# BurnhamG/PyTorch-ScalableFHVAE

Measured on AMD Instinct MI355X. Metric: segments/sec + ELBO (nats/frame), (B,20,80) fbank, higher is better.
Workload: dtype bf16; 1 GPU; c3: fhvae.FHVAE 2x256 LSTM enc/dec, z1=z2=32, 28k-seq mu2 table, batch 2048; per-GPU batch 2048, T=20, F=80, full train step (fwd+loss+bwd+Adam), intended objective, mu_idx uniform; global_batch=2048, parallelism=single

## Files before the change

### include/fhvae_hip.h

```cpp
#ifndef FHVAE_HIP_H
#define FHVAE_HIP_H

#include <stdint.h>

#ifdef __cplusplus
extern "C" {
#endif

#define FHVAE_ABI_VERSION 11

enum { FHVAE_F32 = 0, FHVAE_BF16 = 1 };

enum {
  FHVAE_OK = 0,
  FHVAE_ERR_NULL = -1,
  FHVAE_ERR_SHAPE = -2,
  FHVAE_ERR_DTYPE = -3,
  FHVAE_ERR_ALIGN = -4,
  FHVAE_ERR_LIMIT = -5
};

#define FHVAE_MAX_LAYERS 4
#define FHVAE_LSTM_SYNC_BYTES 16384

// ... 68 lines not shown
int64_t fhvae_lstm_ws_below_elems(const fhvae_lstm_desc* d);
int fhvae_lstm_form(const fhvae_lstm_desc* d);
int fhvae_lstm_seq_fwd(const fhvae_lstm_desc* d, void* stream);
int64_t fhvae_lstm_infer_cs_elems(const fhvae_lstm_desc* d);
int fhvae_lstm_seq_infer(const fhvae_lstm_desc* d, void* stream);

typedef struct fhvae_lstm_bwd_desc {
  fhvae_lstm_desc f;
  const float* d_hs_top;
  const float* d_hn;
  void* dgates;
  float* dgsum;
  float* dc;
  float* dw_ih[FHVAE_MAX_LAYERS];
  float* dw_hh[FHVAE_MAX_LAYERS];
  float* db_ih[FHVAE_MAX_LAYERS];
  float* db_hh[FHVAE_MAX_LAYERS];
  float* d_xc;
  int32_t phase;
  float* ws_below;
} fhvae_lstm_bwd_desc;

int fhvae_lstm_seq_bwd(const fhvae_lstm_bwd_desc* d, void* stream);
typedef struct fhvae_wgrad_desc {
  const void* a; int64_t lda;
  int64_t a_col0;
  const void* b; int64_t ldb;
  float* c; int64_t ldc;
  int64_t M, N, K;
} fhvae_wgrad_desc;
int fhvae_wgrad_desc_ok(const fhvae_wgrad_desc* p);
int fhvae_lstm_param_grads_multi(const fhvae_lstm_bwd_desc* const* descs, int n, const fhvae_wgrad_desc* extra, int n_extra,
                                 void* stream);
int fhvae_wgrad_bf16(const void* a, int64_t lda, const void* b, int64_t ldb, float* c, int64_t ldc, int64_t M,
                     int64_t N, int64_t K, void* stream);
int fhvae_wgrad_f32(const float* a, int64_t lda, const float* b, int64_t ldb, float* c, int64_t ldc, int64_t M, int64_t N,
                    int64_t K, void* stream);

int fhvae_proj_bf16(const void* a, int64_t lda, const void* b, int64_t ldb, const float* bias, float* c, int64_t ldc,
                    int64_t M, int64_t N, int64_t K, void* stream);

int fhvae_mu2_gather_fwd(const float* table, const int64_t* idx, int64_t idx_offset, float* mu2,
                         int64_t B, int64_t S, int64_t D, int32_t* oob_flag, void* stream);
int fhvae_mu2_gather_bwd(const float* dmu2, const int64_t* idx, int64_t idx_offset, float* dtable,
                         int64_t B, int64_t S, int64_t D, float scale, void* stream);

typedef struct fhvae_elbo_desc {
  int64_t B, T, F, D1, D2;
  const float* x;    int64_t x_sb, x_st;
  const float* x_mu; const float* x_lv; int64_t xo_sb, xo_st;
  const float* z1_mu; const float* z1_lv;
  const float* z2_mu; const float* z2_lv;
  const float* mu2;
  const int64_t* num_segs; double nsegs_scalar;
  float* lower_bound; float* log_px_z; float* neg_kld_z1; float* neg_kld_z2; float* log_pmu2;
} fhvae_elbo_desc;

int fhvae_elbo_fwd(const fhvae_elbo_desc* d, void* stream);

typedef struct fhvae_elbo_bwd_desc {
  fhvae_elbo_desc f;
  const float* g_lower_bound; const float* g_log_px_z; const float* g_neg_kld_z1;
  const float* g_neg_kld_z2; const float* g_log_pmu2;
  int32_t reference_detach;
  float* d_x_mu; float* d_x_lv;
  float* d_z1_mu; float* d_z1_lv; float* d_z2_mu; float* d_z2_lv; float* d_mu2;
// ... 85 lines not shown
```

### pytorch-scalablefhvae_amd/csrc/lstm.hip

```cpp
#include "gemm_launch.h"
#include "lstm_cell.h"
#include "lstm_cluster.h"
#include "wgrad.h"
#include "wgrad_f32.h"
#include <algorithm>
#include <vector>
#include "trace.h"
#include <cstdlib>

namespace fh {

constexpr int kCH = 32;

struct GateRowMap {
  int H;
  __device__ __forceinline__ int64_t operator()(int n) const {
    int unit = (n >> 6) * 16 + (n & 15);
    int gate = (n & 63) >> 4;
    return unit < H ? (int64_t)gate * H + unit : -1;
  }
  __device__ __forceinline__ bool all_valid(int n0, int n) const { return ((n0 + n) >> 6) * 16 <= H; }
};

template <typename T>
// ... 683 lines not shown
    return FHVAE_OK;
  }
  for (int64_t w = 0; w < T_ + L - 1; ++w) {
    int nj = 0;
    const BwdJobs<T> jobs = bwd_jobs<T>(bd, op, w, nj);
    double fl = 0;
    for (int j = 0; j < nj; ++j) fl += 2.0 * B * H * (jobs.job[j].seg[0].K + jobs.job[j].seg[1].K);
    const int ts = trace_begin(st, kTraceBwdCell, fl);
    const int bt = B >= 16384 ? 128 : 32;
    if (bt == 128) {
      dim3 grid((unsigned)fh_cdiv(B, 128), (unsigned)fh_cdiv(H, 64), (unsigned)nj);
      hipLaunchKernelGGL((lstm_bwd_step_kernel<T, 128, 64, 4, 1, 16>), grid, dim3(kThreads), 0, st, jobs);
    } else if (bt == 64) {
      dim3 grid((unsigned)fh_cdiv(B, 64), (unsigned)fh_cdiv(H, 64), (unsigned)nj);
      hipLaunchKernelGGL((lstm_bwd_step_kernel<T, 64, 64, 2, 2, 16>), grid, dim3(kThreads), 0, st, jobs);
    } else if (B >= 1024) {
      dim3 grid((unsigned)fh_cdiv(B, 32), (unsigned)fh_cdiv(H, 32), (unsigned)nj);
      hipLaunchKernelGGL((lstm_bwd_step_kernel<T, 32, 32, 2, 2, 16>), grid, dim3(kThreads), 0, st, jobs);
    } else {
      dim3 grid((unsigned)fh_cdiv(B, 32), (unsigned)fh_cdiv(H, 32), (unsigned)nj);
      hipLaunchKernelGGL((lstm_bwd_step_kernel<T, 32, 32, 2, 2, kCH>), grid, dim3(kThreads), 0, st, jobs);
    }
    trace_end(st, ts);
    int e = fh_launch_status();
    if (e) return e;
  }
  return FHVAE_OK;
}

constexpr int64_t kWgradMinK = 1024;

template <typename T>
static int lstm_param_grads(const fhvae_lstm_bwd_desc* bd, const Ops<T>& op, hipStream_t st, std::vector<WgProblem>* wq = nullptr,
                            std::vector<GemmParams>* fq = nullptr, std::vector<WgProblem32>* wq32 = nullptr) {
  const fhvae_lstm_desc* d = &bd->f;
  const int64_t B = d->B, T_ = d->T, I = d->I, Ic = d->Ic, H = d->H;
  const int L = d->L;
  const int64_t K0 = I + Ic, G = 4 * H;
  const T* dg = (const T*)bd->dgates;
  const T* hs = (const T*)d->hs;
  GemmParams grp[2 * FHVAE_MAX_LAYERS];
  int ng = 0;
  auto wgrad_long = [&](const void* a, int64_t lda, const void* b, int64_t ldb, int64_t Kc, float* c, int64_t ldc, int64_t Ncols) {
    if (sizeof(T) == 4) {
      if (!wq32 || Kc < kWgradMinK) return false;
      WgProblem32 w = {};
      w.A = (const float*)a, w.B = (const float*)b, w.C = c;
      w.lda = lda, w.ldb = ldb, w.ldc = ldc;
      w.M = (int)G, w.N = (int)Ncols, w.K = (int)Kc;
      if (!wgrad32_eligible(w)) return false;
      wq32->push_back(w);
      return true;
    }
    if (!wq || sizeof(T) != 2 || Kc < kWgradMinK) return false;
    WgProblem w = {};
    w.A = (const u16*)a, w.B = (const u16*)b, w.C = c;
    w.lda = lda, w.ldb = ldb, w.ldc = ldc;
    w.M = (int)G, w.N = (int)Ncols, w.K = (int)Kc;
    if (!wgrad_eligible(w)) return false;
    wq->push_back(w);
    return true;
  };
  auto wgrad = [&](const void* a, int64_t lda, const void* b, int64_t ldb, int64_t Kc, float* c, int64_t ldc, int64_t Ncols) {
    GemmParams p = {};
    p.seg[0] = Seg{a, lda, 0, b, ldb, 0, (int)Kc, 0};
    p.M = (int)G;
    p.N = (int)Ncols;
    p.C = c;
    p.ldc = ldc;
    p.splitk = 0;
    p.mode = 1;
    return p;
  };
  auto flush = [&]() -> int {
    int e = FHVAE_OK;
    for (int i = 0; i < ng && !e; i += kMaxGroup) e = launch_gemm_group(grp + i, ng - i < kMaxGroup ? ng - i : kMaxGroup, d->dtype, st);
    ng = 0;
    return e;
  };
  for (int l = 0; l < L; ++l) {
    const T* dgl = dg + (int64_t)l * T_ * B * G;
    const T* hl = hs + (int64_t)l * T_ * B * H;
    int e;
    if (bd->dw_hh[l] && T_ > 1 && !wgrad_long(dgl + B * G, G, hl, H, (T_ - 1) * B, bd->dw_hh[l], H, H))
      grp[ng++] = wgrad(dgl + B * G, G, hl, H, (T_ - 1) * B, bd->dw_hh[l], H, H);
    if (bd->dw_ih[l]) {
      if (l > 0) {
        if (!wgrad_long(dgl, G, hs + (int64_t)(l - 1) * T_ * B * H, H, T_ * B, bd->dw_ih[l], H, H))
          grp[ng++] = wgrad(dgl, G, hs + (int64_t)(l - 1) * T_ * B * H, H, T_ * B, bd->dw_ih[l], H, H);
      } else {
        if (I > 0 && !wgrad_long(dgl, G, op.x, I, T_ * B, bd->dw_ih[0], K0, I))
          grp[ng++] = wgrad(dgl, G, op.x, I, T_ * B, bd->dw_ih[0], K0, I);
        if (Ic > 0) {
          GemmParams p = wgrad(bd->dgsum, G, d->xc, Ic, B, bd->dw_ih[0] + I, K0, Ic);
          if (fq) {
            fq->push_back(p);
          } else {
            e = launch_gemm(p, FHVAE_F32, st);
            if (e) return e;
          }
        }
      }
    }
    if (!(sizeof(T) == 2 && cluster_eligible(d))) {
      if (l == 0 && Ic > 0 && bd->dgsum)
        e = launch_colsum(bd->dgsum, FHVAE_F32, G, bd->db_ih[l], bd->db_hh[l], B, G, st);
      else
        e = launch_colsum(dgl, d->dtype, G, bd->db_ih[l], bd->db_hh[l], T_ * B, G, st);
      if (e) return e;
    }
  }
  return flush();
}

static int lstm_dxc(const fhvae_lstm_bwd_desc* bd, hipStream_t st, bool zeroed = false) {
  const fhvae_lstm_desc* d = &bd->f;
  if (!bd->d_xc || d->Ic <= 0) return FHVAE_OK;
  const int64_t G = 4 * d->H, K0 = d->I + d->Ic;
  GemmParams p = {};
  p.seg[0] = Seg{bd->dgsum, G, 1, d->w_ih[0] + d->I, K0, 0, (int)G, 0};
  p.M = (int)d->B;
  p.N = (int)d->Ic;
  p.C = bd->d_xc;
  p.ldc = d->Ic;
  const int64_t tiles = fh_cdiv(d->B, 64) * fh_cdiv(d->Ic, 64);
  if (tiles <= 64 && G >= 512) {
    const int64_t n = d->B * d->Ic;
    if (!zeroed) hipLaunchKernelGGL(zero_f32_kernel, dim3((unsigned)fh_cdiv(n, 1024)), dim3(256), 0, st, bd->d_xc, n);
    p.mode = 2;
    int64_t sk = 256 / tiles;
    while (sk > 1 && G / sk < 128) sk >>= 1;
    p.splitk = (int)(sk < 4 ? 4 : sk > 16 ? 16 : sk);
  } else {
    p.splitk = 1;
  }
  return launch_gemm(p, FHVAE_F32, st);
}
// ... 25 lines not shown
    return launch_wgrad32(wq32.data(), (int)wq32.size(), st);
  }
  Ops<u16> op = ops_bf16(d);
  if (rec) {
    e = lstm_bwd_impl<u16>(bd, op, st);
    if (e) return e;
    e = lstm_dxc(bd, st, cluster_eligible(d) && cluster_bwd_zeroes_dxc(d));
    if (e) return e;
  }
  if (!par) return FHVAE_OK;
  std::vector<WgProblem> wq;
  e = lstm_param_grads<u16>(bd, op, st, getenv("FHVAE_NO_WGRAD") ? nullptr : &wq);
  if (e) return e;
  return launch_wgrad(wq.data(), (int)wq.size(), st);
}

static bool wg_from_desc(const fhvae_wgrad_desc* x, WgProblem& p) {
  if (!x || x->M <= 0 || x->N <= 0 || x->K <= 0 || x->M > INT32_MAX || x->N > INT32_MAX || x->K > INT32_MAX || x->a_col0 < 0 ||
      x->a_col0 > INT32_MAX)
    return false;
  p = WgProblem{};
  p.A = (const u16*)x->a, p.B = (const u16*)x->b, p.C = x->c;
  p.lda = x->lda, p.ldb = x->ldb, p.ldc = x->ldc;
  p.M = (int)x->M, p.N = (int)x->N, p.K = (int)x->K;
  p.a_col0 = (int)x->a_col0;
  return wgrad_eligible(p) && x->ldc >= x->N;
}

extern "C" int fhvae_wgrad_desc_ok(const fhvae_wgrad_desc* x) {
  WgProblem p;
  return wg_from_desc(x, p) ? 1 : 0;
}

extern "C" int fhvae_lstm_param_grads_multi(const fhvae_lstm_bwd_desc* const* bds, int n, const fhvae_wgrad_desc* extra, int n_extra,
                                            void* stream) {
  if (n < 0 || n_extra < 0) return FHVAE_ERR_SHAPE;
  if (n > 0) FH_CHECK_PTR(bds);
  if (n_extra > 0) FH_CHECK_PTR(extra);
  hipStream_t st = (hipStream_t)stream;
  std::vector<WgProblem> wq;
  for (int i = 0; i < n_extra; ++i) {
    WgProblem p;
    if (!wg_from_desc(extra + i, p)) return FHVAE_ERR_ALIGN;
    wq.push_back(p);
  }
  std::vector<GemmParams> fq;
  std::vector<WgProblem32> wq32;
  const bool use_wq = !getenv("FHVAE_NO_WGRAD");
  for (int i = 0; i < n; ++i) {
    const fhvae_lstm_bwd_desc* bd = bds[i];
    FH_CHECK_PTR(bd);
    const fhvae_lstm_desc* d = &bd->f;
    int e = check_desc(d);
    if (e) return e;
    FH_CHECK_PTR(bd->dgates);
    if (d->Ic > 0) FH_CHECK_PTR(bd->dgsum);
    if (d->dtype == FHVAE_F32) {
      e = lstm_param_grads<float>(bd, ops_f32(d), st, nullptr, nullptr, use_wq ? &wq32 : nullptr);
    } else {
      e = lstm_param_grads<u16>(bd, ops_bf16(d), st, use_wq ? &wq : nullptr, &fq);
    }
    if (e) return e;
  }
  for (size_t i = 0; i < fq.size();) {
    size_t j = i;
    while (j < fq.size() && j - i < (size_t)kMaxGroup) {
      bool dup = false;
      for (size_t k = i; k < j; ++k) dup = dup || fq[k].C == fq[j].C;
      if (dup) break;
      ++j;
    }
    const int e = launch_gemm_group(fq.data() + i, (int)(j - i), FHVAE_F32, st);
    if (e) return e;
    i = j;
  }
  {
    const int e = launch_wgrad32(wq32.data(), (int)wq32.size(), st);
    if (e) return e;
  }
  return launch_wgrad(wq.data(), (int)wq.size(), st);
}
```

### pytorch-scalablefhvae_amd/csrc/wgrad.h

```cpp
#pragma once
#include "common.h"

namespace fh {

struct WgProblem {
  const u16* A;
  const u16* B;
  float* C;
  int64_t lda, ldb, ldc;
  int M, N, K;
  int m_tiles, n_tiles, splitk, ksteps_per;
  int shared_c;
  int a_col0;
};

constexpr int kMaxWgProblems = 16;
struct WgGroup {
  int n;
  int base[kMaxWgProblems + 1];
  WgProblem p[kMaxWgProblems];
};

bool wgrad_eligible(const WgProblem& p);
int launch_wgrad(const WgProblem* ps, int n, hipStream_t st);

}
```

### pytorch-scalablefhvae_amd/csrc/wgrad.hip

```cpp
#include "wgrad.h"

#include <algorithm>
#include <cstdlib>

#include "gemm_core.h"

namespace fh {

constexpr int kWgThreads = 512;
constexpr int kWgBM = 256, kWgBK = 64;

template <int W>
struct WgImg {
  static constexpr int RB = W * 2;
  static constexpr int BYTES = kWgBK * RB;
  static constexpr int CPR = RB / 16;
  static constexpr int RPI = 1024 / RB;
  static constexpr int NI = BYTES / 1024 / 8;
};

typedef void __attribute__((address_space(3))) * lds_void_p;

template <int W>
__device__ __forceinline__ void wg_dma_offsets(unsigned (&voff)[WgImg<W>::NI], unsigned ld_bytes, int wave, int lane) {
  using I = WgImg<W>;
#pragma unroll
  for (int q = 0; q < I::NI; ++q) {
    const int row = (wave * I::NI + q) * I::RPI + lane / I::CPR;
    const int pc = lane % I::CPR;
    const int c = ((((pc >> 1) ^ (row & 7)) << 1) | (pc & 1));
    voff[q] = (unsigned)row * ld_bytes + (unsigned)c * 16u;
  }
}

template <int W>
__device__ __forceinline__ void wg_issue(char* stage, __amdgpu_buffer_rsrc_t rs, const unsigned (&voff)[WgImg<W>::NI], unsigned kbase,
                                         int wave) {
  using I = WgImg<W>;
#pragma unroll
  for (int q = 0; q < I::NI; ++q)
    __builtin_amdgcn_raw_ptr_buffer_load_lds(rs, (lds_void_p)(stage + (wave * I::NI + q) * 1024), 16, voff[q] + kbase, 0, 0, 0);
}

template <int RB>
__device__ __forceinline__ bf16x8 wg_frag(const char* img, int off, int j) {
  typedef s16x4 __attribute__((address_space(3))) * lds_p;
  const char* a0 = img + off + j * 32 * RB;
  union {
    struct {
      s16x4 lo, hi;
    } s;
    bf16x8 v;
  } u;
  u.s.lo = __builtin_amdgcn_ds_read_tr16_b64_v4i16((lds_p)(a0));
  u.s.hi = __builtin_amdgcn_ds_read_tr16_b64_v4i16((lds_p)(a0 + 16 * RB));
  return u.v;
}

template <int BN>
__global__ __launch_bounds__(kWgThreads) void wgrad_kernel(WgGroup g) {
  using IA = WgImg<kWgBM>;
  using IB = WgImg<BN>;
  constexpr int STAGE = IA::BYTES + IB::BYTES;
  constexpr int TM = 8, TN = BN / 64;
  constexpr int NLOAD = IA::NI + IB::NI;
  __shared__ __attribute__((aligned(1024))) char stage0[STAGE];
  __shared__ __attribute__((aligned(1024))) char stage1[STAGE];

  int wg = blockIdx.x;
  {
    const int nb = gridDim.x;
    if (nb >= 16) {
      const int q = nb >> 3, r = nb & 7, xcd = wg & 7;
      wg = (xcd < r ? xcd * (q + 1) : r * (q + 1) + (xcd - r) * q) + (wg >> 3);
    }
  }
  int pi = 0;
  while (pi + 1 < g.n && wg >= g.base[pi + 1]) ++pi;
  const WgProblem& p = g.p[pi];
  const int local = wg - g.base[pi];
  const int mt = local % p.m_tiles, nt = (local / p.m_tiles) % p.n_tiles, sp = local / (p.m_tiles * p.n_tiles);
  const int ks_total = (p.K + kWgBK - 1) / kWgBK;
  const int ks0 = sp * p.ksteps_per, ks1 = min(ks_total, ks0 + p.ksteps_per);
  if (ks0 >= ks1) return;
  const int m0 = mt * kWgBM, n0 = nt * BN;

  const int tid = threadIdx.x, lane = tid & 63, wave = tid >> 6;
  const int wm = wave >> 2, wn = wave & 3;
  const int gq = lane >> 4, i = lane & 15;

  const unsigned lda_b = (unsigned)p.lda * 2u, ldb_b = (unsigned)p.ldb * 2u;
  const __amdgpu_buffer_rsrc_t rsa =
      __builtin_amdgcn_make_buffer_rsrc(const_cast<u16*>(p.A + m0), 0, (int)(((int64_t)p.K * p.lda - p.a_col0 - m0) * 2), 0x00020000);
  const __amdgpu_buffer_rsrc_t rsb =
      __builtin_amdgcn_make_buffer_rsrc(const_cast<u16*>(p.B + n0), 0, (int)(((int64_t)p.K * p.ldb - n0) * 2), 0x00020000);
  unsigned va[IA::NI], vb[IB::NI];
  wg_dma_offsets<kWgBM>(va, lda_b, wave, lane);
  wg_dma_offsets<BN>(vb, ldb_b, wave, lane);
  auto a_step = [&](int ks) -> unsigned { return (unsigned)(ks * kWgBK) * lda_b; };

  const int kr = 4 * gq + (i >> 2), x = kr & 7;
  int offa[TM], offb[TN];
#pragma unroll
  for (int tm = 0; tm < TM; ++tm) offa[tm] = kr * IA::RB + ((((wm * 8 + tm)) ^ x) << 5) + 8 * (i & 3);
#pragma unroll
  for (int tn = 0; tn < TN; ++tn) offb[tn] = kr * IB::RB + ((((wn * TN + tn)) ^ x) << 5) + 8 * (i & 3);

  f32x4 acc[TM][TN];
#pragma unroll
  for (int tm = 0; tm < TM; ++tm)
#pragma unroll
    for (int tn = 0; tn < TN; ++tn) acc[tm][tn] = f32x4{0.f, 0.f, 0.f, 0.f};

  constexpr unsigned kOob = 0x40000000u;
  auto issue = [&](char* st, int ks) {
    const bool in = ks < ks1;
    wg_issue<kWgBM>(st, rsa, va, in ? a_step(ks) : kOob, wave);
// ... 6 lines not shown
      bf16x8 a[TM], b[TN];
#pragma unroll
      for (int tn = 0; tn < TN; ++tn) b[tn] = wg_frag<IB::RB>(Bs, offb[tn], j);
#pragma unroll
      for (int tm = 0; tm < TM; ++tm) a[tm] = wg_frag<IA::RB>(As, offa[tm], j);
      {
        const bool in = ks_next < ks1;
        if (j == 0)
          wg_issue<kWgBM>(nxt, rsa, va, in ? a_step(ks_next) : kOob, wave);
        else
          wg_issue<BN>(nxt + IA::BYTES, rsb, vb, in ? (unsigned)(ks_next * kWgBK) * ldb_b : kOob, wave);
      }
      __builtin_amdgcn_s_setprio(1);
#pragma unroll
      for (int tm = 0; tm < TM; ++tm)
#pragma unroll
        for (int tn = 0; tn < TN; ++tn) acc[tm][tn] = __builtin_amdgcn_mfma_f32_16x16x32_bf16(a[tm], b[tn], acc[tm][tn], 0, 0, 0);
      __builtin_amdgcn_s_setprio(0);
    }
  };
  auto step = [&](const char* cur, char* nxt, int ks_next) {
    asm volatile("s_waitcnt vmcnt(0)" ::: "memory");
    __builtin_amdgcn_s_barrier();
    compute(cur, nxt, ks_next);
    __builtin_amdgcn_s_barrier();
  };
  issue(stage0, ks0);
  for (int ks = ks0; ks < ks1; ks += 2) {
    step(stage0, stage1, ks + 1);
    step(stage1, stage0, ks + 2);
  }
  asm volatile("s_waitcnt vmcnt(0)" ::: "memory");

#pragma unroll
  for (int tm = 0; tm < TM; ++tm)
#pragma unroll
    for (int tn = 0; tn < TN; ++tn) {
      const int n = n0 + wn * (BN / 4) + tn * 16 + i;
#pragma unroll
      for (int r = 0; r < 4; ++r) {
        const int m = m0 + wm * 128 + tm * 16 + 4 * gq + r;
        if (m < p.M && n < p.N) {
          float* c = p.C + (int64_t)m * p.ldc + n;
          if (p.splitk == 1 && !p.shared_c)
            *c += acc[tm][tn][r];
          else
            atomicAdd(c, acc[tm][tn][r]);
        }
      }
    }
}

template __global__ void wgrad_kernel<256>(WgGroup);
template __global__ void wgrad_kernel<128>(WgGroup);

bool wgrad_eligible(const WgProblem& p) {
  if (p.M <= 0 || p.N <= 0 || p.K <= 0 || !p.A || !p.B || !p.C) return false;
  if ((((uintptr_t)p.A) | ((uintptr_t)p.B)) & 15) return false;
  if ((p.lda % 8) || (p.ldb % 8) || p.lda < p.a_col0 + p.M || p.ldb < p.N || p.a_col0 < 0) return false;
  if ((int64_t)p.K * p.lda * 2 >= (1LL << 30) || (int64_t)p.K * p.ldb * 2 >= (1LL << 30)) return false;
  return true;
}

template <int BN>
static int launch_class(const WgProblem* ps, const int* which, int n, hipStream_t st) {
  for (int at = 0; at < n; at += kMaxWgProblems) {
    const int cnt = n - at < kMaxWgProblems ? n - at : kMaxWgProblems;
    int64_t tiles = 0;
    for (int k = 0; k < cnt; ++k) {
      const WgProblem& p = ps[which[at + k]];
      tiles += fh_cdiv(p.M, kWgBM) * fh_cdiv(p.N, BN);
    }
    int64_t ks_max = 1;
    for (int k = 0; k < cnt; ++k) ks_max = std::max<int64_t>(ks_max, fh_cdiv(ps[which[at + k]].K, kWgBK));
    const double t_step = 2.0 * kWgBM * BN * kWgBK / (1.0e15 / 256), tile_bytes = 4.0 * kWgBM * BN;
    int64_t sk = 1;
    double best = 1e30;
    for (int64_t c = 1; c <= 64 && c * 2 <= ks_max; ++c) {
      const double waves = (double)fh_cdiv(tiles * c, 256), steps = (double)fh_cdiv(ks_max, c) + 2.0;
      const double t = waves * steps * t_step + (c > 1 ? tiles * c * tile_bytes / 1.3e12 : 0.0);
      if (t < best) best = t, sk = c;
    }
    WgGroup g = {};
    g.n = cnt;
    for (int k = 0; k < cnt; ++k) {
      WgProblem p = ps[which[at + k]];
      p.m_tiles = (int)fh_cdiv(p.M, kWgBM);
      p.n_tiles = (int)fh_cdiv(p.N, BN);
      const int64_t ks_total = fh_cdiv(p.K, kWgBK);
      int64_t s = sk;
      if (s > ks_total / 2) s = ks_total / 2;
      if (s < 1) s = 1;
      p.ksteps_per = (int)fh_cdiv(ks_total, s);
      p.splitk = (int)fh_cdiv(ks_total, p.ksteps_per);
      g.p[k] = p;
      g.base[k + 1] = g.base[k] + p.m_tiles * p.n_tiles * p.splitk;
    }
    for (int a = 0; a < cnt; ++a)
      for (int b = 0; b < cnt; ++b)
        if (a != b && g.p[a].C == g.p[b].C) g.p[a].shared_c = 1;
    const dim3 grid((unsigned)g.base[cnt]), block(kWgThreads);
    hipLaunchKernelGGL((wgrad_kernel<BN>), grid, block, 0, st, g);
    const int e = fh_launch_status();
    if (e) return e;
  }
  return FHVAE_OK;
}

int launch_wgrad(const WgProblem* ps, int n, hipStream_t st) {
  if (n <= 0) return FHVAE_OK;
  int wide[256], narrow[256], nw = 0, nn = 0;
  if (n > 256) return FHVAE_ERR_LIMIT;
  for (int k = 0; k < n; ++k) {
    if (!wgrad_eligible(ps[k])) return FHVAE_ERR_ALIGN;
    if (ps[k].N > 128)
      wide[nw++] = k;
    else
      narrow[nn++] = k;
  }
  int e = launch_class<256>(ps, wide, nw, st);
  if (e) return e;
  return launch_class<128>(ps, narrow, nn, st);
}

}

using namespace fh;

extern "C" int fhvae_wgrad_bf16(const void* a, int64_t lda, const void* b, int64_t ldb, float* c, int64_t ldc, int64_t M, int64_t N,
                                int64_t K, void* stream) {
  FH_CHECK_PTR(a);
  FH_CHECK_PTR(b);
  FH_CHECK_PTR(c);
  FH_CHECK_POS(M);
  FH_CHECK_POS(N);
  FH_CHECK_POS(K);
  FH_CHECK_I32(M);
  FH_CHECK_I32(N);
  FH_CHECK_I32(K);
  WgProblem p = {};
  p.A = (const u16*)a, p.B = (const u16*)b, p.C = c;
  p.lda = lda, p.ldb = ldb, p.ldc = ldc;
  p.M = (int)M, p.N = (int)N, p.K = (int)K;
  if (!wgrad_eligible(p)) return FHVAE_ERR_ALIGN;
  return launch_wgrad(&p, 1, (hipStream_t)stream);
}
```

### pytorch-scalablefhvae_amd/hip_binding.py

```python
from __future__ import annotations

import ctypes as C
import os
from typing import List, Optional, Sequence

import numpy as np
import torch

_HERE = os.path.dirname(os.path.abspath(__file__))
LIB_PATH = os.path.join(_HERE, "libfhvae_hip.so")

F32, BF16 = 0, 1
MAX_LAYERS = 4
ABI_VERSION = 11
PZ2_LOGVAR = np.log(0.5 ** 2).astype(np.float32)
INV_TWO_VAR = float(np.float32(1.0) / (np.float32(2.0) * np.exp(PZ2_LOGVAR)))

_vp, _i64, _i32, _f32, _f64 = C.c_void_p, C.c_int64, C.c_int32, C.c_float, C.c_double


class LstmDesc(C.Structure):
    _fields_ = [
        ("dtype", _i32), ("L", _i32),
        ("B", _i64), ("T", _i64), ("I", _i64), ("Ic", _i64), ("H", _i64),
# ... 43 lines not shown
class WgradDesc(C.Structure):
    _fields_ = [("a", _vp), ("lda", _i64), ("a_col0", _i64), ("b", _vp), ("ldb", _i64), ("c", _vp), ("ldc", _i64),
                ("M", _i64), ("N", _i64), ("K", _i64)]


SIGNATURES = {
    "fhvae_abi_version": (C.c_int, []),
    "fhvae_strerror": (C.c_char_p, [C.c_int]),
    "fhvae_linear_fwd": (C.c_int, [_vp, _i64, _vp, _i64, _vp, _vp, _i64, _vp, _i64, _i64, _i64, C.c_int, C.c_int, _vp]),
    "fhvae_linear_bwd": (C.c_int, [_vp, _i64, _vp, _i64, _vp, _i64, _vp, _i64, _vp, _vp, _i64, _vp, _i64, _vp, _i64, _i64,
                                   _i64, C.c_int, C.c_int, _vp]),
    "fhvae_gauss_head_reparam_fwd": (C.c_int, [_vp, _i64, _vp, _vp, _vp, _vp, _vp, _vp, _vp, _vp, _i64, _i64, _i64, C.c_int,
                                               _vp]),
    "fhvae_gauss_head_pair_fwd": (C.c_int, [_vp, _i64, _vp, _vp, _vp, _vp, _i64, _i64, _i64, _i64, _vp]),
    "fhvae_gauss_reparam_bwd": (C.c_int, [_vp, _vp, _vp, _vp, _vp, _vp, _vp, _i64, _vp]),
    "fhvae_gauss_head_bwd": (C.c_int, [_vp, _i64, _vp, _vp, _vp, _vp, _vp, _vp, _vp, _vp, _vp, _i64, _vp, _vp, _vp, _vp, _i64, _i64, _i64, _vp]),
    "fhvae_head_pair_weights": (C.c_int, [_vp, _vp, _vp, _vp, _i64, _i64, _i64, _vp]),
    "fhvae_gauss_reparam_pair_fwd": (C.c_int, [_vp, _i64, _vp, _vp, _vp, _vp, _i64, _i64, _vp]),
    "fhvae_gauss_reparam_bwd_pair": (C.c_int, [_vp, _vp, _vp, _i64, _vp, _vp, _i64, _vp, _i64, _vp, _vp, _i64, _i64, _vp]),
    "fhvae_elbo_colsum_rows": (_i64, [_i64]),
    "fhvae_gauss_head_bwd_pair": (C.c_int, [_vp, _i64, _vp, _i64, _vp, _i64, _vp, _i64, _vp, _i64, _vp, _vp, _vp, _vp, _i64, _i64, _i64, _vp]),
    "fhvae_loss_fwd": (C.c_int, [_vp, _vp, _f32, _vp, _i64, _vp, _vp]),
    "fhvae_loss_bwd": (C.c_int, [_vp, _f32, _vp, _vp, _i64, _vp]),
    "fhvae_lstm_lp_bytes": (_i64, [C.POINTER(LstmDesc)]),
    "fhvae_lstm_form": (C.c_int, [C.POINTER(LstmDesc)]),
    "fhvae_lstm_layout_id": (C.c_int, [C.POINTER(LstmDesc)]),
    "fhvae_lstm_pre_elems": (_i64, [C.POINTER(LstmDesc)]),
    "fhvae_lstm_ws_below_elems": (_i64, [C.POINTER(LstmDesc)]),
    "fhvae_lstm_seq_fwd": (C.c_int, [C.POINTER(LstmDesc), _vp]),
    "fhvae_lstm_infer_cs_elems": (_i64, [C.POINTER(LstmDesc)]),
    "fhvae_lstm_seq_infer": (C.c_int, [C.POINTER(LstmDesc), _vp]),
    "fhvae_lstm_seq_bwd": (C.c_int, [C.POINTER(LstmBwdDesc), _vp]),
    "fhvae_lstm_param_grads_multi": (C.c_int, [_vp, C.c_int, _vp, C.c_int, _vp]),
    "fhvae_wgrad_desc_ok": (C.c_int, [_vp]),
    "fhvae_wgrad_bf16": (C.c_int, [_vp, _i64, _vp, _i64, _vp, _i64, _i64, _i64, _i64, _vp]),
    "fhvae_wgrad_f32": (C.c_int, [_vp, _i64, _vp, _i64, _vp, _i64, _i64, _i64, _i64, _vp]),
    "fhvae_proj_bf16": (C.c_int, [_vp, _i64, _vp, _i64, _vp, _vp, _i64, _i64, _i64, _i64, _vp]),
    "fhvae_mu2_gather_fwd": (C.c_int, [_vp, _vp, _i64, _vp, _i64, _i64, _i64, _vp, _vp]),
    "fhvae_mu2_gather_bwd": (C.c_int, [_vp, _vp, _i64, _vp, _i64, _i64, _i64, _f32, _vp]),
    "fhvae_shard_pack": (C.c_int, [_vp, _vp, _vp, _i64, _i64, _vp]),
    "fhvae_shard_unpack": (C.c_int, [_vp, _vp, _vp, _i64, _i64, _vp]),
    "fhvae_disc_merge_partials": (C.c_int, [_vp, _vp, _vp, _vp, _i64, _i64, _vp]),
    "fhvae_shard_bwd_pack": (C.c_int, [_vp, _f32, _vp, _i64, _i64, _vp, _i64, _i64, _vp]),
    "fhvae_shard_bwd_unpack": (C.c_int, [_vp, _i64, _i64, _vp, _vp, _i64, _i64, _vp]),
    "fhvae_disc_ce_mean": (C.c_int, [_vp, _vp, _vp, _vp, _f32, _i64, _vp]),
    "fhvae_elbo_fwd": (C.c_int, [C.POINTER(ElboDesc), _vp]),
    "fhvae_elbo_bwd": (C.c_int, [C.POINTER(ElboBwdDesc), _vp]),
    "fhvae_disc_lse_ws_bytes": (_i64, [_i64, _i64]),
    "fhvae_disc_lse_bwd_ws_bytes": (_i64, [_i64, _i64, _i64]),
    "fhvae_disc_lse_fwd": (C.c_int, [_vp, _vp, _vp, _i64, _f32, _vp, _vp, _vp, _vp, _f32, _vp, _i64, _i64, _i64, C.c_int, _vp]),
    "fhvae_disc_lse_bwd": (C.c_int, [_vp, _vp, _vp, _i64, _f32, _vp, _vp, _vp, _f32, _vp, _vp, _vp, _i64, _i64, _i64, _i64, C.c_int, _vp]),
    "fhvae_adam_step": (C.c_int, [_vp, _vp, _vp, _vp, _vp, _i64, _f32, _f32, _f32, _f32, _f32, C.c_int, _vp, _vp]),
    "fhvae_segment_gather": (C.c_int, [_vp, _i64, _vp, _vp, _vp, _vp, _vp, _i64, _i64, _i64, _vp, _vp]),
    "fhvae_mu2_accumulate": (C.c_int, [_vp, _vp, _vp, _vp, _i64, _i64, _i64, _vp]),
    "fhvae_mu2_finalize": (C.c_int, [_vp, _vp, _vp, _i64, _i64, _f32, _vp]),
    "fhvae_hs_select": (C.c_int, [_vp, _i64, _vp, _i64, _vp, _vp, _vp, _i64, _vp, _vp]),
    "fhvae_mu2_accumulate_sorted": (C.c_int, [_vp, _vp, _vp, _vp, _i64, _i64, _i64, _vp, _vp]),
    "fhvae_mu2_load_table": (C.c_int, [_vp, _vp, _vp, _vp, _vp, _i64, _i64, _f32, _vp]),
    "fhvae_hs_pack_partials": (C.c_int, [_vp, _vp, _vp, _i64, _i64, _vp]),
    "fhvae_mu2_merge_load_shard": (C.c_int, [_vp, _i64, _i64, _i64, _i64, _vp, _vp, _vp, _i64, _f32, _vp]),
    "fhvae_feats_tile_rows": (C.c_int, [_i64, C.c_int]),
    "fhvae_feats_fwd": (C.c_int, [_vp, _i64, _vp, _vp, _i64, _i64, _vp, _vp, _i64, _i64, _i64, C.c_int, _vp, _vp, _vp]),
    "fhvae_trace_enable": (C.c_int, [C.c_int]),
    "fhvae_trace_collect": (_i64, [_vp, _vp, _vp, _i64]),
    "fhvae_to_time_major": (C.c_int, [_vp, _vp, _vp, _i64, _i64, _i64, C.c_int, _vp]),
    "fhvae_cast_bf16": (C.c_int, [_vp, _vp, _vp, _i64, _i64, _vp]),
}

_lib = None


def load_library(path: str = LIB_PATH):
    global _lib
    if _lib is not None:
        return _lib
    if not os.path.exists(path):
        raise RuntimeError(
            "libfhvae_hip.so is not built (%s). Run `python pytorch-scalablefhvae_amd/build_ext.py` "
            "(or __graft_entry__.build()). There is no CPU fallback." % path
        )
    lib = C.CDLL(path)
    for name, (res, args) in SIGNATURES.items():
        fn = getattr(lib, name)
        fn.restype = res
        fn.argtypes = args
    if lib.fhvae_abi_version() != ABI_VERSION:
        raise RuntimeError("libfhvae_hip.so ABI version mismatch")
    _lib = lib
    return lib


_SIDE = {"stream": None, "pending": False, "keep": [], "enabled": False}


LSTM_BWD_REC_HOOK = {"fn": None}


_DEFER = {"enabled": not os.environ.get("FHVAE_NO_DEFER"), "pending": [], "extra": []}


def flush_param_grads():
    pend, extra = _DEFER["pending"], _DEFER["extra"]
    if not pend and not extra:
        return
    lib = load_library()
    n, nx = len(pend), len(extra)
    arr = (C.POINTER(LstmBwdDesc) * n)(*[C.pointer(bd) for bd, _ in pend]) if n else None
    xs = (WgradDesc * nx)(*[x for x, _ in extra]) if nx else None
    with _Timed("fhvae_lstm_param_grads_multi"):
        _check(lib.fhvae_lstm_param_grads_multi(arr, n, xs, nx, _stream()), "fhvae_lstm_param_grads_multi")
    pend.clear()
    extra.clear()


def flush_param_grads_except_last():
    pend = _DEFER["pending"]
    if len(pend) <= 1:
        return
    last = pend.pop()
    flush_param_grads()
    pend.append(last)


def set_defer_param_grads(on: bool):
    flush_param_grads()
    _DEFER["enabled"] = bool(on)


def side_stream():
    if _SIDE["stream"] is None:
        _SIDE["stream"] = torch.cuda.Stream()
    return _SIDE["stream"]


def join_side_stream():
    if _SIDE["pending"]:
        torch.cuda.current_stream().wait_stream(_SIDE["stream"])
        _SIDE["pending"] = False
        _SIDE["keep"].clear()


def set_side_stream_enabled(on: bool):
    join_side_stream()
# ... 1130 lines not shown
```

Measured before the change: 1.243 million segments/s.

## Rework bf16 wgrad planning with slab split-K reduction, pairing, and unified launch

Replaces the per-width wgrad launches with a single kernel that handles both 128- and 256-wide tiles. A new cost-model planner picks per-problem split-K slice counts. Overlapping problems that share A/B with a row offset are paired so they schedule together. Split-K partials are written to a workspace slab and summed by a separate reduce kernel, instead of being accumulated into C with atomics. Python allocates and caches the workspace per device. This trades an extra reduce launch and workspace traffic for fewer atomics, better load balance and fewer launches.

```diff
diff --git a/include/fhvae_hip.h b/include/fhvae_hip.h
--- a/include/fhvae_hip.h
+++ b/include/fhvae_hip.h
@@ -124,6 +124,9 @@
 int fhvae_wgrad_desc_ok(const fhvae_wgrad_desc* p);
 int fhvae_lstm_param_grads_multi(const fhvae_lstm_bwd_desc* const* descs, int n, const fhvae_wgrad_desc* extra, int n_extra,
                                  void* stream);
+int64_t fhvae_lstm_param_grads_ws_bytes(const fhvae_lstm_bwd_desc* const* descs, int n, const fhvae_wgrad_desc* extra, int n_extra);
+int fhvae_lstm_param_grads_multi_ws(const fhvae_lstm_bwd_desc* const* descs, int n, const fhvae_wgrad_desc* extra, int n_extra,
+                                    void* ws, int64_t ws_bytes, void* stream);
 int fhvae_wgrad_bf16(const void* a, int64_t lda, const void* b, int64_t ldb, float* c, int64_t ldc, int64_t M,
                      int64_t N, int64_t K, void* stream);
 int fhvae_wgrad_f32(const float* a, int64_t lda, const float* b, int64_t ldb, float* c, int64_t ldc, int64_t M, int64_t N,
diff --git a/pytorch-scalablefhvae_amd/csrc/lstm.hip b/pytorch-scalablefhvae_amd/csrc/lstm.hip
--- a/pytorch-scalablefhvae_amd/csrc/lstm.hip
+++ b/pytorch-scalablefhvae_amd/csrc/lstm.hip
@@ -739,7 +739,7 @@
 
 template <typename T>
 static int lstm_param_grads(const fhvae_lstm_bwd_desc* bd, const Ops<T>& op, hipStream_t st, std::vector<WgProblem>* wq = nullptr,
-                            std::vector<GemmParams>* fq = nullptr, std::vector<WgProblem32>* wq32 = nullptr) {
+                            std::vector<GemmParams>* fq = nullptr, std::vector<WgProblem32>* wq32 = nullptr, bool dry = false) {
   const fhvae_lstm_desc* d = &bd->f;
   const int64_t B = d->B, T_ = d->T, I = d->I, Ic = d->Ic, H = d->H;
   const int L = d->L;
@@ -780,6 +780,7 @@
     return p;
   };
   auto flush = [&]() -> int {
+    if (dry) return FHVAE_OK;
     int e = FHVAE_OK;
     for (int i = 0; i < ng && !e; i += kMaxGroup) e = launch_gemm_group(grp + i, ng - i < kMaxGroup ? ng - i : kMaxGroup, d->dtype, st);
     ng = 0;
@@ -802,14 +803,14 @@
           GemmParams p = wgrad(bd->dgsum, G, d->xc, Ic, B, bd->dw_ih[0] + I, K0, Ic);
           if (fq) {
             fq->push_back(p);
-          } else {
+          } else if (!dry) {
             e = launch_gemm(p, FHVAE_F32, st);
             if (e) return e;
           }
         }
       }
     }
-    if (!(sizeof(T) == 2 && cluster_eligible(d))) {
+    if (!dry && !(sizeof(T) == 2 && cluster_eligible(d))) {
       if (l == 0 && Ic > 0 && bd->dgsum)
         e = launch_colsum(bd->dgsum, FHVAE_F32, G, bd->db_ih[l], bd->db_hh[l], B, G, st);
       else
@@ -901,12 +902,11 @@
   return wg_from_desc(x, p) ? 1 : 0;
 }
 
-extern "C" int fhvae_lstm_param_grads_multi(const fhvae_lstm_bwd_desc* const* bds, int n, const fhvae_wgrad_desc* extra, int n_extra,
-                                            void* stream) {
+static int param_grads_multi(const fhvae_lstm_bwd_desc* const* bds, int n, const fhvae_wgrad_desc* extra, int n_extra, void* ws,
+                             int64_t ws_bytes, bool dry, int64_t* ws_need, hipStream_t st) {
   if (n < 0 || n_extra < 0) return FHVAE_ERR_SHAPE;
   if (n > 0) FH_CHECK_PTR(bds);
   if (n_extra > 0) FH_CHECK_PTR(extra);
-  hipStream_t st = (hipStream_t)stream;
   std::vector<WgProblem> wq;
   for (int i = 0; i < n_extra; ++i) {
     WgProblem p;
@@ -925,11 +925,15 @@
     FH_CHECK_PTR(bd->dgates);
     if (d->Ic > 0) FH_CHECK_PTR(bd->dgsum);
     if (d->dtype == FHVAE_F32) {
-      e = lstm_param_grads<float>(bd, ops_f32(d), st, nullptr, nullptr, use_wq ? &wq32 : nullptr);
+      e = lstm_param_grads<float>(bd, ops_f32(d), st, nullptr, nullptr, use_wq ? &wq32 : nullptr, dry);
     } else {
-      e = lstm_param_grads<u16>(bd, ops_bf16(d), st, use_wq ? &wq : nullptr, &fq);
+      e = lstm_param_grads<u16>(bd, ops_bf16(d), st, use_wq ? &wq : nullptr, &fq, nullptr, dry);
     }
     if (e) return e;
+  }
+  if (dry) {
+    *ws_need = wgrad_ws_bytes(wq.data(), (int)wq.size());
+    return FHVAE_OK;
   }
   for (size_t i = 0; i < fq.size();) {
     size_t j = i;
@@ -947,5 +951,23 @@
     const int e = launch_wgrad32(wq32.data(), (int)wq32.size(), st);
     if (e) return e;
   }
-  return launch_wgrad(wq.data(), (int)wq.size(), st);
-}
+  return launch_wgrad(wq.data(), (int)wq.size(), st, ws, ws_bytes);
+}
+
+extern "C" int fhvae_lstm_param_grads_multi(const fhvae_lstm_bwd_desc* const* bds, int n, const fhvae_wgrad_desc* extra, int n_extra,
+                                            void* stream) {
+  return param_grads_multi(bds, n, extra, n_extra, nullptr, 0, false, nullptr, (hipStream_t)stream);
+}
+
+extern "C" int64_t fhvae_lstm_param_grads_ws_bytes(const fhvae_lstm_bwd_desc* const* bds, int n, const fhvae_wgrad_desc* extra,
+                                                   int n_extra) {
+  int64_t need = 0;
+  const int e = param_grads_multi(bds, n, extra, n_extra, nullptr, 0, true, &need, nullptr);
+  return e ? (e < 0 ? e : -e) : need;
+}
+
+extern "C" int fhvae_lstm_param_grads_multi_ws(const fhvae_lstm_bwd_desc* const* bds, int n, const fhvae_wgrad_desc* extra, int n_extra,
+                                               void* ws, int64_t ws_bytes, void* stream) {
+  if (ws_bytes < 0) return FHVAE_ERR_SHAPE;
+  return param_grads_multi(bds, n, extra, n_extra, ws, ws_bytes, false, nullptr, (hipStream_t)stream);
+}
diff --git a/pytorch-scalablefhvae_amd/csrc/wgrad.h b/pytorch-scalablefhvae_amd/csrc/wgrad.h
--- a/pytorch-scalablefhvae_amd/csrc/wgrad.h
+++ b/pytorch-scalablefhvae_amd/csrc/wgrad.h
@@ -12,16 +12,22 @@
   int m_tiles, n_tiles, splitk, ksteps_per;
   int shared_c;
   int a_col0;
+  int bn;
+  int pair;
+  int k_shift;
+  int64_t slab;
 };
 
-constexpr int kMaxWgProblems = 16;
+constexpr int kMaxWgProblems = 24;
 struct WgGroup {
   int n;
   int base[kMaxWgProblems + 1];
+  float* ws;
   WgProblem p[kMaxWgProblems];
 };
 
 bool wgrad_eligible(const WgProblem& p);
-int launch_wgrad(const WgProblem* ps, int n, hipStream_t st);
+int launch_wgrad(const WgProblem* ps, int n, hipStream_t st, void* ws = nullptr, int64_t ws_bytes = 0);
+int64_t wgrad_ws_bytes(const WgProblem* ps, int n);
 
 }
diff --git a/pytorch-scalablefhvae_amd/csrc/wgrad.hip b/pytorch-scalablefhvae_amd/csrc/wgrad.hip
--- a/pytorch-scalablefhvae_amd/csrc/wgrad.hip
+++ b/pytorch-scalablefhvae_amd/csrc/wgrad.hip
@@ -34,8 +34,7 @@
 }
 
 template <int W>
-__device__ __forceinline__ void wg_issue(char* stage, __amdgpu_buffer_rsrc_t rs, const unsigned (&voff)[WgImg<W>::NI], unsigned kbase,
-                                         int wave) {
+__device__ __forceinline__ void wg_issue(char* stage, __amdgpu_buffer_rsrc_t rs, const unsigned* voff, unsigned kbase, int wave) {
   using I = WgImg<W>;
 #pragma unroll
   for (int q = 0; q < I::NI; ++q)
@@ -58,31 +57,14 @@
 }
 
 template <int BN>
-__global__ __launch_bounds__(kWgThreads) void wgrad_kernel(WgGroup g) {
+__device__ __forceinline__ void wg_tile(const WgProblem& p, int mt, int nt, int sp, char* stage0, char* stage1,
+                                                              float* ws) {
   using IA = WgImg<kWgBM>;
   using IB = WgImg<BN>;
-  constexpr int STAGE = IA::BYTES + IB::BYTES;
   constexpr int TM = 8, TN = BN / 64;
-  constexpr int NLOAD = IA::NI + IB::NI;
-  __shared__ __attribute__((aligned(1024))) char stage0[STAGE];
-  __shared__ __attribute__((aligned(1024))) char stage1[STAGE];
-
-  int wg = blockIdx.x;
-  {
-    const int nb = gridDim.x;
-    if (nb >= 16) {
-      const int q = nb >> 3, r = nb & 7, xcd = wg & 7;
-      wg = (xcd < r ? xcd * (q + 1) : r * (q + 1) + (xcd - r) * q) + (wg >> 3);
-    }
-  }
-  int pi = 0;
-  while (pi + 1 < g.n && wg >= g.base[pi + 1]) ++pi;
-  const WgProblem& p = g.p[pi];
-  const int local = wg - g.base[pi];
-  const int mt = local % p.m_tiles, nt = (local / p.m_tiles) % p.n_tiles, sp = local / (p.m_tiles * p.n_tiles);
   const int ks_total = (p.K + kWgBK - 1) / kWgBK;
-  const int ks0 = sp * p.ksteps_per, ks1 = min(ks_total, ks0 + p.ksteps_per);
-  if (ks0 >= ks1) return;
+  const int ks_lo = sp * p.ksteps_per - p.k_shift, ks1 = min(ks_total, ks_lo + p.ksteps_per), ks0 = max(ks_lo, 0);
+  if (ks0 >= ks1 && p.slab < 0) return;
   const int m0 = mt * kWgBM, n0 = nt * BN;
 
   const int tid = threadIdx.x, lane = tid & 63, wave = tid >> 6;
@@ -155,6 +137,15 @@
   }
   asm volatile("s_waitcnt vmcnt(0)" ::: "memory");
 
+  if (p.slab >= 0) {
+    f32x4* s = reinterpret_cast<f32x4*>(ws + p.slab + (int64_t)((sp * p.n_tiles + nt) * p.m_tiles + mt) * (kWgBM * BN)) +
+               wave * (TM * TN * 64) + lane;
+#pragma unroll
+    for (int tm = 0; tm < TM; ++tm)
+#pragma unroll
+      for (int tn = 0; tn < TN; ++tn) s[(tm * TN + tn) * 64] = acc[tm][tn];
+    return;
+  }
 #pragma unroll
   for (int tm = 0; tm < TM; ++tm)
 #pragma unroll
@@ -174,8 +165,99 @@
     }
 }
 
-template __global__ void wgrad_kernel<256>(WgGroup);
-template __global__ void wgrad_kernel<128>(WgGroup);
+constexpr int kWgStage = WgImg<kWgBM>::BYTES * 2;
+
+__global__ __launch_bounds__(kWgThreads) void wgrad_kernel(WgGroup g) {
+  __shared__ __attribute__((aligned(1024))) char stage0[kWgStage];
+  __shared__ __attribute__((aligned(1024))) char stage1[kWgStage];
+
+  int wg = blockIdx.x;
+  {
+    const int nb = gridDim.x;
+    if (nb >= 16) {
+      const int q = nb >> 3, r = nb & 7, xcd = wg & 7;
+      wg = (xcd < r ? xcd * (q + 1) : r * (q + 1) + (xcd - r) * q) + (wg >> 3);
+    }
+  }
+  int pi = 0;
+  while (pi + 1 < g.n && wg >= g.base[pi + 1]) ++pi;
+  int local = wg - g.base[pi];
+  const int tiles = g.p[pi].m_tiles * g.p[pi].n_tiles;
+  int sp;
+  if (g.p[pi].pair) {
+    sp = local / (2 * tiles);
+    local -= sp * 2 * tiles;
+    if (local >= tiles) local -= tiles, ++pi;
+  } else {
+    sp = local / tiles;
+    local -= sp * tiles;
+  }
+  const WgProblem& p = g.p[pi];
+  const int mt = local % p.m_tiles, nt = local / p.m_tiles;
+  if (p.bn == 256)
+    wg_tile<256>(p, mt, nt, sp, stage0, stage1, g.ws);
+  else
+    wg_tile<128>(p, mt, nt, sp, stage0, stage1, g.ws);
+}
+
+constexpr int kMaxWgRedSrc = 4;
+struct WgRedEntry {
+  float* C;
+  int64_t slab[kMaxWgRedSrc];
+  int64_t ldc;
+  int M, N, bn, m_tiles, tiles, np;
+  int splits[kMaxWgRedSrc];
+};
+struct WgRed {
+  int n;
+  int base[kMaxWgProblems + 1];
+  const float* ws;
+  WgRedEntry e[kMaxWgProblems];
+};
+
+__global__ __launch_bounds__(256) void wgrad_reduce_kernel(WgRed r) {
+  const int b = blockIdx.x;
+  int ei = 0;
+  while (ei + 1 < r.n && b >= r.base[ei + 1]) ++ei;
+  const WgRedEntry& e = r.e[ei];
+  const int per_tile = kWgBM * e.bn / 4;
+  const int idx = (b - r.base[ei]) * 256 + (int)threadIdx.x;
+  const int t = idx / per_tile, f = idx - t * per_tile;
+  const int lane = f & 63, frag = f >> 6;
+  const int TN = e.bn / 64;
+  const int wave = frag / (8 * TN), tmn = frag - wave * 8 * TN, tm = tmn / TN, tn = tmn - tm * TN;
+  const int wm = wave >> 2, wn = wave & 3, gq = lane >> 4, i = lane & 15;
+  const int mt = t % e.m_tiles, nt = t / e.m_tiles;
+  const int n = nt * e.bn + wn * (e.bn / 4) + tn * 16 + i;
+  const int m = mt * kWgBM + wm * 128 + tm * 16 + 4 * gq;
+  const int64_t stride = (int64_t)e.tiles * per_tile;
+  f32x4 v = {0.f, 0.f, 0.f, 0.f};
+  for (int j = 0; j < e.np; ++j) {
+    const f32x4* s = reinterpret_cast<const f32x4*>(r.ws + e.slab[j]) + idx;
+    for (int k0 = 0; k0 < e.splits[j]; k0 += 8) {
+      f32x4 x[8];
+#pragma unroll
+      for (int u = 0; u < 8; ++u)
+        if (k0 + u < e.splits[j]) x[u] = __builtin_nontemporal_load(s + (k0 + u) * stride);
+#pragma unroll
+      for (int u = 0; u < 8; ++u)
+        if (k0 + u < e.splits[j]) v += x[u];
+    }
+  }
+  if (n < e.N) {
+    const int rows = min(4, e.M - m);
+    float* c = e.C + (int64_t)m * e.ldc + n;
+    if (rows == 4) {
+      float x[4];
+#pragma unroll
+      for (int q = 0; q < 4; ++q) x[q] = c[q * e.ldc];
+#pragma unroll
+      for (int q = 0; q < 4; ++q) c[q * e.ldc] = x[q] + v[q];
+    } else {
+      for (int q = 0; q < rows; ++q) c[q * e.ldc] += v[q];
+    }
+  }
+}
 
 bool wgrad_eligible(const WgProblem& p) {
   if (p.M <= 0 || p.N <= 0 || p.K <= 0 || !p.A || !p.B || !p.C) return false;
@@ -185,65 +267,179 @@
   return true;
 }
 
-template <int BN>
-static int launch_class(const WgProblem* ps, const int* which, int n, hipStream_t st) {
-  for (int at = 0; at < n; at += kMaxWgProblems) {
-    const int cnt = n - at < kMaxWgProblems ? n - at : kMaxWgProblems;
-    int64_t tiles = 0;
+constexpr int kWgCUs = 256;
+constexpr double kWgNarrowStep = 0.6;
+
+static double wg_step_cost(const WgProblem& p) { return p.bn == 256 ? 1.0 : kWgNarrowStep; }
+
+static void wg_slices(const WgProblem& p, double tau, int64_t& kp, int64_t& s) {
+  const int64_t ks = fh_cdiv(p.K, kWgBK);
+  int64_t kmax = (int64_t)(tau / wg_step_cost(p) + 1e-9) - 2;
+  if (kmax < 1) kmax = 1;
+  s = std::min<int64_t>(fh_cdiv(ks, kmax), std::max<int64_t>(1, ks / 2));
+  kp = fh_cdiv(ks, s);
+  s = fh_cdiv(ks, kp);
+}
+
+static void wg_plan_slices(WgProblem* q, int n, bool slab) {
+  const double t_step = 2.0 * kWgBM * 256 * kWgBK / (1.0e15 / kWgCUs);
+  const double rate = slab ? 2.5e12 : 1.3e12;
+  std::vector<double> cand;
+  for (int k = 0; k < n; ++k) {
+    if (k > 0 && q[k - 1].pair) continue;
+    const int64_t ks = fh_cdiv(q[k].K, kWgBK);
+    for (int c = 1; c <= 64; ++c) cand.push_back((double)(fh_cdiv(ks, c) + 2) * wg_step_cost(q[k]));
+  }
+  std::sort(cand.begin(), cand.end());
+  cand.erase(std::unique(cand.begin(), cand.end()), cand.end());
+  double best = 1e30, best_tau = cand.empty() ? 1.0 : cand[0];
+  for (double tau : cand) {
+    int64_t wgs = 0;
+    double longest = 0, partial = 0;
+    for (int k = 0; k < n; ++k) {
+      if (k > 0 && q[k - 1].pair) continue;
+      int64_t kp, s;
+      wg_slices(q[k], tau, kp, s);
+      const int64_t units = (int64_t)q[k].m_tiles * q[k].n_tiles * s * (q[k].pair ? 2 : 1);
+      wgs += units;
+      longest = std::max(longest, (double)(kp + 2) * wg_step_cost(q[k]));
+      if (s > 1 || q[k].shared_c || (q[k].pair && q[k + 1].shared_c)) partial += (double)units * 4.0 * kWgBM * q[k].bn;
+    }
+    const double t = (double)fh_cdiv(wgs, kWgCUs) * longest * t_step + partial / rate + (slab && partial > 0 ? 3e-6 : 0.0);
+    if (t < best) best = t, best_tau = tau;
+  }
+  for (int k = 0; k < n; ++k) {
+    if (k > 0 && q[k - 1].pair) {
+      q[k].ksteps_per = q[k - 1].ksteps_per, q[k].splitk = q[k - 1].splitk;
+      continue;
+    }
+    int64_t kp, s;
+    wg_slices(q[k], best_tau, kp, s);
+    q[k].ksteps_per = (int)kp, q[k].splitk = (int)s;
+  }
+}
+
+static bool wg_pairable(const WgProblem& f, const WgProblem& s, int& shift) {
+  if (f.bn != s.bn || f.M != s.M || f.N != s.N || f.lda != s.lda || f.a_col0 != s.a_col0 || f.C == s.C) return false;
+  const intptr_t d = (intptr_t)s.A - (intptr_t)f.A, row = (intptr_t)f.lda * 2;
+  if (d <= 0 || d % row) return false;
+  const int64_t rows = d / row;
+  if (rows % kWgBK || (int64_t)s.K + rows != (int64_t)f.K) return false;
+  shift = (int)(rows / kWgBK);
+  return true;
+}
+
+struct WgLaunch {
+  WgGroup g;
+  WgRed red;
+};
+
+static void wg_build(const WgProblem* ps, int n, bool slab, std::vector<WgLaunch>& out, int64_t& ws_floats) {
+  std::vector<WgProblem> q(ps, ps + n);
+  for (WgProblem& p : q) {
+    p.bn = p.N > 128 ? 256 : 128;
+    p.m_tiles = (int)fh_cdiv(p.M, kWgBM);
+    p.n_tiles = (int)fh_cdiv(p.N, p.bn);
+    p.pair = 0, p.k_shift = 0, p.shared_c = 0, p.slab = -1;
+  }
+  std::vector<int> partner(n, -1), shift(n, 0);
+  for (int i = 0; i < n; ++i)
+    for (int j = 0; j < n && partner[i] < 0; ++j)
+      if (j != i && partner[j] < 0 && wg_pairable(q[i], q[j], shift[j])) partner[i] = j, partner[j] = i, shift[i] = -1;
+  std::vector<WgProblem> o;
+  std::vector<char> placed(n, 0);
+  for (int i = 0; i < n; ++i) {
+    if (placed[i]) continue;
+    if (partner[i] < 0) {
+      o.push_back(q[i]), placed[i] = 1;
+      continue;
+    }
+    const int f = shift[i] < 0 ? i : partner[i], s = partner[f];
+    WgProblem a = q[f], b = q[s];
+    a.pair = 1, b.k_shift = shift[s];
+    o.push_back(a), o.push_back(b), placed[f] = placed[s] = 1;
+  }
+  ws_floats = 0;
+  out.clear();
+  for (int at = 0; at < n;) {
+    int cnt = std::min(n - at, kMaxWgProblems);
+    if (o[at + cnt - 1].pair) --cnt;
+    WgProblem* c = o.data() + at;
+    for (int x = 0; x < cnt; ++x)
+      for (int y = 0; y < cnt; ++y)
+        if (x != y && c[x].C == c[y].C) c[x].shared_c = 1;
+    WgLaunch L = {};
+    bool use_slab = slab;
+    for (int pass = 0; pass < 2; ++pass) {
+      wg_plan_slices(c, cnt, use_slab);
+      L.red = WgRed{};
+      int64_t off = 0;
+      bool ok = true;
+      for (int k = 0; k < cnt; ++k) {
+        WgProblem& p = c[k];
+        p.slab = -1;
+        if (!use_slab || (p.splitk == 1 && !p.shared_c)) continue;
+        p.slab = off;
+        off += (int64_t)p.splitk * p.m_tiles * p.n_tiles * kWgBM * p.bn;
+        int e = 0;
+        while (e < L.red.n && L.red.e[e].C != p.C) ++e;
+        WgRedEntry& r = L.red.e[e];
+        if (e == L.red.n) {
+          ++L.red.n;
+          r.C = p.C, r.ldc = p.ldc, r.M = p.M, r.N = p.N, r.bn = p.bn, r.m_tiles = p.m_tiles, r.tiles = p.m_tiles * p.n_tiles;
+        } else if (r.np == kMaxWgRedSrc || r.ldc != p.ldc || r.M != p.M || r.N != p.N || r.bn != p.bn) {
+          ok = false;
+        }
+        if (ok) r.splits[r.np] = p.splitk, r.slab[r.np++] = p.slab;
+      }
+      if (ok) {
+        if (use_slab) ws_floats = std::max(ws_floats, off);
+        break;
+      }
+      use_slab = false;
+    }
+    L.g.n = cnt;
     for (int k = 0; k < cnt; ++k) {
-      const WgProblem& p = ps[which[at + k]];
-      tiles += fh_cdiv(p.M, kWgBM) * fh_cdiv(p.N, BN);
-    }
-    int64_t ks_max = 1;
-    for (int k = 0; k < cnt; ++k) ks_max = std::max<int64_t>(ks_max, fh_cdiv(ps[which[at + k]].K, kWgBK));
-    const double t_step = 2.0 * kWgBM * BN * kWgBK / (1.0e15 / 256), tile_bytes = 4.0 * kWgBM * BN;
-    int64_t sk = 1;
-    double best = 1e30;
-    for (int64_t c = 1; c <= 64 && c * 2 <= ks_max; ++c) {
-      const double waves = (double)fh_cdiv(tiles * c, 256), steps = (double)fh_cdiv(ks_max, c) + 2.0;
-      const double t = waves * steps * t_step + (c > 1 ? tiles * c * tile_bytes / 1.3e12 : 0.0);
-      if (t < best) best = t, sk = c;
-    }
-    WgGroup g = {};
-    g.n = cnt;
-    for (int k = 0; k < cnt; ++k) {
-      WgProblem p = ps[which[at + k]];
-      p.m_tiles = (int)fh_cdiv(p.M, kWgBM);
-      p.n_tiles = (int)fh_cdiv(p.N, BN);
-      const int64_t ks_total = fh_cdiv(p.K, kWgBK);
-      int64_t s = sk;
-      if (s > ks_total / 2) s = ks_total / 2;
-      if (s < 1) s = 1;
-      p.ksteps_per = (int)fh_cdiv(ks_total, s);
-      p.splitk = (int)fh_cdiv(ks_total, p.ksteps_per);
-      g.p[k] = p;
-      g.base[k + 1] = g.base[k] + p.m_tiles * p.n_tiles * p.splitk;
-    }
-    for (int a = 0; a < cnt; ++a)
-      for (int b = 0; b < cnt; ++b)
-        if (a != b && g.p[a].C == g.p[b].C) g.p[a].shared_c = 1;
-    const dim3 grid((unsigned)g.base[cnt]), block(kWgThreads);
-    hipLaunchKernelGGL((wgrad_kernel<BN>), grid, block, 0, st, g);
-    const int e = fh_launch_status();
+      L.g.p[k] = c[k];
+      const int64_t w = (k > 0 && c[k - 1].pair) ? 0 : (int64_t)c[k].m_tiles * c[k].n_tiles * c[k].splitk * (c[k].pair ? 2 : 1);
+      L.g.base[k + 1] = L.g.base[k] + (int)w;
+    }
+    for (int e = 0; e < L.red.n; ++e) L.red.base[e + 1] = L.red.base[e] + L.red.e[e].tiles * L.red.e[e].bn / 4;
+    out.push_back(L);
+    at += cnt;
+  }
+}
+
+int64_t wgrad_ws_bytes(const WgProblem* ps, int n) {
+  if (n <= 0 || n > 256) return 0;
+  std::vector<WgLaunch> ls;
+  int64_t f = 0;
+  wg_build(ps, n, true, ls, f);
+  return f * 4;
+}
+
+int launch_wgrad(const WgProblem* ps, int n, hipStream_t st, void* ws, int64_t ws_bytes) {
+  if (n <= 0) return FHVAE_OK;
+  if (n > 256) return FHVAE_ERR_LIMIT;
+  for (int k = 0; k < n; ++k)
+    if (!wgrad_eligible(ps[k])) return FHVAE_ERR_ALIGN;
+  std::vector<WgLaunch> ls;
+  int64_t f = 0;
+  const bool slab = ws && !((uintptr_t)ws & 15);
+  wg_build(ps, n, slab, ls, f);
+  if (slab && f * 4 > ws_bytes) wg_build(ps, n, false, ls, f);
+  for (WgLaunch& L : ls) {
+    L.g.ws = static_cast<float*>(ws);
+    hipLaunchKernelGGL(wgrad_kernel, dim3((unsigned)L.g.base[L.g.n]), dim3(kWgThreads), 0, st, L.g);
+    int e = fh_launch_status();
     if (e) return e;
+    if (L.red.n == 0) continue;
+    L.red.ws = static_cast<const float*>(ws);
+    hipLaunchKernelGGL(wgrad_reduce_kernel, dim3((unsigned)L.red.base[L.red.n]), dim3(256), 0, st, L.red);
+    e = fh_launch_status();
+    if (e) return e;
   }
   return FHVAE_OK;
-}
-
-int launch_wgrad(const WgProblem* ps, int n, hipStream_t st) {
-  if (n <= 0) return FHVAE_OK;
-  int wide[256], narrow[256], nw = 0, nn = 0;
-  if (n > 256) return FHVAE_ERR_LIMIT;
-  for (int k = 0; k < n; ++k) {
-    if (!wgrad_eligible(ps[k])) return FHVAE_ERR_ALIGN;
-    if (ps[k].N > 128)
-      wide[nw++] = k;
-    else
-      narrow[nn++] = k;
-  }
-  int e = launch_class<256>(ps, wide, nw, st);
-  if (e) return e;
-  return launch_class<128>(ps, narrow, nn, st);
 }
 
 }
diff --git a/pytorch-scalablefhvae_amd/hip_binding.py b/pytorch-scalablefhvae_amd/hip_binding.py
--- a/pytorch-scalablefhvae_amd/hip_binding.py
+++ b/pytorch-scalablefhvae_amd/hip_binding.py
@@ -99,6 +99,8 @@
     "fhvae_lstm_seq_infer": (C.c_int, [C.POINTER(LstmDesc), _vp]),
     "fhvae_lstm_seq_bwd": (C.c_int, [C.POINTER(LstmBwdDesc), _vp]),
     "fhvae_lstm_param_grads_multi": (C.c_int, [_vp, C.c_int, _vp, C.c_int, _vp]),
+    "fhvae_lstm_param_grads_ws_bytes": (_i64, [_vp, C.c_int, _vp, C.c_int]),
+    "fhvae_lstm_param_grads_multi_ws": (C.c_int, [_vp, C.c_int, _vp, C.c_int, _vp, _i64, _vp]),
     "fhvae_wgrad_desc_ok": (C.c_int, [_vp]),
     "fhvae_wgrad_bf16": (C.c_int, [_vp, _i64, _vp, _i64, _vp, _i64, _i64, _i64, _i64, _vp]),
     "fhvae_wgrad_f32": (C.c_int, [_vp, _i64, _vp, _i64, _vp, _i64, _i64, _i64, _i64, _vp]),
@@ -164,6 +166,18 @@
 
 
 _DEFER = {"enabled": not os.environ.get("FHVAE_NO_DEFER"), "pending": [], "extra": []}
+_WGRAD_WS = {}
+
+
+def _wgrad_ws(lib, arr, n, xs, nx):
+    held = _WGRAD_WS.setdefault(torch.cuda.current_device(), [])
+    if not torch.cuda.is_current_stream_capturing():
+        need = lib.fhvae_lstm_param_grads_ws_bytes(arr, n, xs, nx)
+        if need < 0:
+            _check(int(need), "fhvae_lstm_param_grads_ws_bytes")
+        if need > 0 and (not held or held[-1].numel() < need):
+            held.append(torch.empty(need, dtype=torch.uint8, device="cuda"))
+    return (held[-1].data_ptr(), held[-1].numel()) if held else (None, 0)
 
 
 def flush_param_grads():
@@ -174,8 +188,9 @@
     n, nx = len(pend), len(extra)
     arr = (C.POINTER(LstmBwdDesc) * n)(*[C.pointer(bd) for bd, _ in pend]) if n else None
     xs = (WgradDesc * nx)(*[x for x, _ in extra]) if nx else None
+    ws, ws_bytes = _wgrad_ws(lib, arr, n, xs, nx)
     with _Timed("fhvae_lstm_param_grads_multi"):
-        _check(lib.fhvae_lstm_param_grads_multi(arr, n, xs, nx, _stream()), "fhvae_lstm_param_grads_multi")
+        _check(lib.fhvae_lstm_param_grads_multi_ws(arr, n, xs, nx, ws, ws_bytes, _stream()), "fhvae_lstm_param_grads_multi")
     pend.clear()
     extra.clear()
 
```

After: 1.259 million segments/s, median of 6. 1.3% higher.
